# pytorch/ELF

Hardware: AMD Instinct MI355X
Metric: mcts_rollouts_per_sec (self-play, 19x19 Go, 8192 rollouts/move, bs 16) (higher is better)
Workload: dtype f32; 1 GPU; BASELINE configs[2]: MCTS self-play bs=16, 8192 rollouts/move, 20x256 fp16 net on PyTorch-ROCm, 2048 games/GPU in 1 group(s), window crosses a move boundary; games_per_gpu=2048, groups=1, board_size=19, mcts_threads=1, net_dtype=fp16, moves_in_window=2048, nodes_per_game=12288, node_bytes=6626, live_nodes=6241478, largest_tree=8184

## Files before the change

### elf_amd/csrc/net_conv3x3.hip

```cpp
#include <hip/hip_runtime.h>
#include <stdint.h>

#include <atomic>

#include "../../include/elf_amd.h"


namespace {

typedef _Float16 half8 __attribute__((ext_vector_type(8)));
typedef _Float16 half4 __attribute__((ext_vector_type(4)));
typedef float floatx16 __attribute__((ext_vector_type(16)));

constexpr int kTileM = 256;
constexpr int kTileN = 256;
constexpr int kThreads = 512;
constexpr int kOperandBytes = 256 * 128;
constexpr int kBufBytes = 2 * kOperandBytes;
constexpr int kWaveCBytes = 4096;
constexpr int kLdsBytes = 2 * kBufBytes + 8 * kWaveCBytes;

__device__ __attribute__((aligned(128))) unsigned char g_zero_line[128] = {0};

typedef const __attribute__((address_space(1))) void* gptr_t;
typedef __attribute__((address_space(3))) void* lptr_t;

__device__ __forceinline__ void stage16(const char* src, char* lds_base) {
  __builtin_amdgcn_global_load_lds((gptr_t)src, (lptr_t)lds_base, 16, 0, 0);
}

template <int kN, bool kLgkm>
__device__ __forceinline__ void wait_staged() {
  if constexpr (kLgkm) asm volatile("s_waitcnt vmcnt(%0) lgkmcnt(0)" ::"n"(kN) : "memory");
  else asm volatile("s_waitcnt vmcnt(%0)" ::"n"(kN) : "memory");
}
__device__ __forceinline__ void raw_barrier() {
  __builtin_amdgcn_s_barrier();
  asm volatile("" ::: "memory");
  __builtin_amdgcn_sched_barrier(0);
}
template <int kV> struct Mode { static constexpr int v = kV; };
__device__ __forceinline__ int fresh(int v) {
  asm volatile("" : "+v"(v));
  return v;
}
__device__ __forceinline__ int fresh_uniform(int v) {
  asm volatile("" : "+s"(v));
  return v;
}

struct WorkItem { int tile, col, half; };
__host__ __device__ inline WorkItem work_item(int id, int tiles, int nfull) {
  int half = -1;
  if (id >= nfull) {
    const int e = id - nfull;
    id = nfull + (e >> 1);
    half = e & 1;
  }
  const int col = id / tiles;
  return WorkItem{id - col * tiles, col, half};
}
__host__ __device__ inline int full_items(int64_t total, int64_t width) {
  const int64_t r = total % width;
  return (int)(total >= width && r > 0 && 2 * r <= width ? total - r : total);
}

struct Ctx {
  char* lds;
  const char* x;
  const char* w;
  int M, H, W, Cin, K, relu;
  int lane, wv;
  const unsigned char* zsrc;
};
struct Rows { uint32_t xoff[4], woff[4], xmask[4]; };

template <int kNT>
__device__ __forceinline__ void decode_rows(const Ctx& c, Rows& rw, int tile, int kbase) {
  const int lane = c.lane, wv = c.wv;
  const int hw = fresh_uniform(c.H * c.W), wd = fresh_uniform(c.W);
#pragma unroll
  for (int j = 0; j < 4; ++j) {
    const int hf = j >> 1, i = j & 1;
    const int r = i * 128 + hf * 64 + wv * 8 + (lane >> 3);
    const int p = tile * kTileM + r;
    uint32_t m = 0;
    if (p < c.M) {
      const int rem = p % hw, hh = rem / wd, ww = rem - hh * wd;
#pragma unroll
      for (int tap = 0; tap < 9; ++tap) {
        const int dy = tap / 3 - 1, dx = tap % 3 - 1;
        if ((unsigned)(hh + dy) < (unsigned)c.H && (unsigned)(ww + dx) < (unsigned)c.W) m |= 1u << tap;
      }
    }
    rw.xmask[j] = m;
    rw.xoff[j] = (uint32_t)p * (uint32_t)(c.Cin * 2) + (((lane & 7) ^ ((r >> 1) & 7)) << 4);
    const int rwt = kNT == 2 ? (i * 2 + (wv >> 2)) * 64 + hf * 32 + (wv & 3) * 8 + (lane >> 3) : i * 64 + wv * 8 + (lane >> 3);
    rw.woff[j] = (uint32_t)(kbase + rwt) * (uint32_t)(9 * c.Cin * 2) + (((lane & 7) ^ ((rwt >> 1) & 7)) << 4);
  }
}
__device__ __forceinline__ void stage_x(const Ctx& c, const Rows& rw, int hf, int tap, int kc, int buf) {
  const int dy = tap / 3 - 1, dx = tap - (tap / 3) * 3 - 1;
  const uint32_t d = (uint32_t)((dy * c.W + dx) * c.Cin * 2 + kc * 128);
#pragma unroll
  for (int i = 0; i < 2; ++i)
    stage16(((rw.xmask[hf * 2 + i] >> tap) & 1) ? c.x + (uint32_t)(rw.xoff[hf * 2 + i] + d) : (const char*)c.zsrc,
            c.lds + buf * kBufBytes + (i * 128 + hf * 64 + c.wv * 8) * 128);
}
template <int kNT>
__device__ __forceinline__ void stage_w(const Ctx& c, const Rows& rw, int hf, int tap, int kc, int buf) {
  const uint32_t d = (uint32_t)(tap * c.Cin * 2 + kc * 128);
#pragma unroll
  for (int i = 0; i < 2; ++i)
    stage16(c.w + (uint32_t)(rw.woff[hf * 2 + i] + d),
            c.lds + buf * kBufBytes + kOperandBytes +
                (kNT == 2 ? (i * 2 + (c.wv >> 2)) * 64 + hf * 32 + (c.wv & 3) * 8 : i * 64 + c.wv * 8) * 128);
}
struct KPos { int tap1, kc1, tap2, kc2; };
__device__ __forceinline__ KPos first_kpos(int kchunks) {
  KPos k{0, 1, 0, 2};
  if (kchunks == 1) { k.tap1 = 1; k.kc1 = 0; k.tap2 = 2; k.kc2 = 0; }
  else if (kchunks == 2) { k.tap2 = 1; k.kc2 = 0; }
  return k;
}
template <int kNT>
__device__ __forceinline__ void issue_prologue(const Ctx& c, const Rows& rw, int kchunks) {
  const KPos k = first_kpos(fresh_uniform(kchunks));
  stage_x(c, rw, 0, 0, 0, 0); stage_w<kNT>(c, rw, 0, 0, 0, 0);
  if constexpr (kNT == 2) stage_w<kNT>(c, rw, 1, 0, 0, 0);
  stage_x(c, rw, 1, 0, 0, 0);
  stage_x(c, rw, 0, k.tap1, k.kc1, 1); stage_w<kNT>(c, rw, 0, k.tap1, k.kc1, 1);
  if constexpr (kNT == 2) stage_w<kNT>(c, rw, 1, k.tap1, k.kc1, 1);
}

template <int kNT>
__device__ __forceinline__ void main_loop(const Ctx& c, const Rows& rw, floatx16 (&acc)[4][kNT]) {
  char* const lds = c.lds;
  const int lane = c.lane, wv = c.wv;
  const int wm = wv >> 2, wn = wv & 3;
  const int fr = lane & 31, fh = lane >> 5;
  const int sw = (fr >> 1) & 7;
  const int xrow = (wm * 128 + fr) * 128;
  const int wrow = kOperandBytes + (wn * 32 * kNT + fr) * 128;
  int cs[4];
#pragma unroll
  for (int kk = 0; kk < 4; ++kk) cs[kk] = (((kk >> 1) * 4 + fh * 2 + (kk & 1)) ^ sw) << 4;
  auto ldx = [&](const char* b, int mt, int kk) { return *(const half8*)(b + xrow + mt * 4096 + cs[kk]); };
  auto ldw = [&](const char* b, int nt, int kk) { return *(const half8*)(b + wrow + nt * 4096 + cs[kk]); };

#pragma unroll
  for (int mt = 0; mt < 4; ++mt)
#pragma unroll
    for (int nt = 0; nt < kNT; ++nt)
#pragma unroll
      for (int e = 0; e < 16; ++e) acc[mt][nt][e] = 0.0f;

  constexpr int kFly = 2 * (2 + kNT);
  const int kchunks = c.Cin >> 6, ktiles = 9 * kchunks;
  half8 xf[2][4], wa[4], wb[kNT == 2 ? 4 : 1];
  KPos k = first_kpos(kchunks);

  auto ktile = [&](auto mode, int t) {
    constexpr int kMode = decltype(mode)::v;
    const int cur = t & 1, nxt = cur ^ 1;
    const char* b = lds + cur * kBufBytes;
#pragma unroll
    for (int kk = 0; kk < 4; ++kk) {
      wa[kk] = ldw(b, 0, kk);
      xf[0][kk] = ldx(b, 0, kk);
      xf[1][kk] = ldx(b, 1, kk);
      if constexpr (kNT == 2) wb[kk] = ldw(b, 1, kk);
    }
    if constexpr (kMode <= 1) stage_x(c, rw, 1, k.tap1, k.kc1, nxt);
    wait_staged<kMode == 2 ? 0 : kFly, true>();
    raw_barrier();
    __builtin_amdgcn_s_setprio(1);
#pragma unroll
    for (int kk = 0; kk < 4; ++kk) {
      acc[0][0] = __builtin_amdgcn_mfma_f32_32x32x16_f16(wa[kk], xf[0][kk], acc[0][0], 0, 0, 0);
      acc[1][0] = __builtin_amdgcn_mfma_f32_32x32x16_f16(wa[kk], xf[1][kk], acc[1][0], 0, 0, 0);
      if constexpr (kNT == 2) {
        acc[0][1] = __builtin_amdgcn_mfma_f32_32x32x16_f16(wb[kk], xf[0][kk], acc[0][1], 0, 0, 0);
        acc[1][1] = __builtin_amdgcn_mfma_f32_32x32x16_f16(wb[kk], xf[1][kk], acc[1][1], 0, 0, 0);
      }
    }
    __builtin_amdgcn_s_setprio(0);
    __builtin_amdgcn_sched_barrier(0);
    raw_barrier();
#pragma unroll
    for (int kk = 0; kk < 4; ++kk) {
      xf[0][kk] = ldx(b, 2, kk);
      xf[1][kk] = ldx(b, 3, kk);
    }
    if constexpr (kMode == 0) {
      stage_x(c, rw, 0, k.tap2, k.kc2, cur); stage_w<kNT>(c, rw, 0, k.tap2, k.kc2, cur);
      if constexpr (kNT == 2) stage_w<kNT>(c, rw, 1, k.tap2, k.kc2, cur);
    }
    wait_staged<kMode == 0 ? kFly : kMode == 1 ? 2 : 0, true>();
    raw_barrier();
    __builtin_amdgcn_s_setprio(1);
#pragma unroll
    for (int kk = 0; kk < 4; ++kk) {
      acc[2][0] = __builtin_amdgcn_mfma_f32_32x32x16_f16(wa[kk], xf[0][kk], acc[2][0], 0, 0, 0);
      acc[3][0] = __builtin_amdgcn_mfma_f32_32x32x16_f16(wa[kk], xf[1][kk], acc[3][0], 0, 0, 0);
      if constexpr (kNT == 2) {
        acc[2][1] = __builtin_amdgcn_mfma_f32_32x32x16_f16(wb[kk], xf[0][kk], acc[2][1], 0, 0, 0);
        acc[3][1] = __builtin_amdgcn_mfma_f32_32x32x16_f16(wb[kk], xf[1][kk], acc[3][1], 0, 0, 0);
      }
    }
    __builtin_amdgcn_s_setprio(0);
    __builtin_amdgcn_sched_barrier(0);
    raw_barrier();
  };
  const int late = __builtin_amdgcn_readfirstlane(threadIdx.x >> 8);
  if (late) raw_barrier();
  for (int t = 0; t < ktiles - 2; ++t) {
    ktile(Mode<0>{}, t);
    k.tap1 = k.tap2; k.kc1 = k.kc2;
    if (++k.kc2 == kchunks) { k.kc2 = 0; ++k.tap2; }
  }
  ktile(Mode<1>{}, ktiles - 2);
  ktile(Mode<2>{}, ktiles - 1);
  if (!late) raw_barrier();
}

template <bool kHasRes, int kNT>
struct Skip { half8 bv; half8 rv[kHasRes ? 8 * kNT : 1]; };

template <int kNT>
struct EpiLane {
  static constexpr int kC = 4 * kNT;
  static constexpr int kPos = 64 / kC;
  static constexpr int kR = 32 / kPos;
  int pr, q, chan;
  int row0;
  __device__ __forceinline__ EpiLane(const Ctx& c, int tile, int kbase)
      : pr(c.lane / kC), q(c.lane % kC), chan(kbase + (c.wv & 3) * 32 * kNT + (c.lane % kC) * 8),
        row0(tile * kTileM + (c.wv >> 2) * 128) {}
  static __device__ __forceinline__ int swz(int p) { return kNT == 2 ? (p >> 1) & 7 : (p >> 2) & 3; }
};

template <bool kHasRes, int kNT>
__device__ __forceinline__ void load_bias(const Ctx& c, Skip<kHasRes, kNT>& s, const _Float16* __restrict__ bias, int tile, int kbase) {
  const EpiLane<kNT> e(c, tile, kbase);
  s.bv = *(const half8*)(bias + e.chan);
}
template <bool kHasRes, int kNT>
__device__ __forceinline__ void load_skip(const Ctx& c, Skip<kHasRes, kNT>& s, const _Float16* __restrict__ res, int tile, int kbase) {
  using E = EpiLane<kNT>;
  const E e(c, tile, kbase);
  if constexpr (kHasRes) {
#pragma unroll
    for (int it = 0; it < 4 * E::kR; ++it) {
      const int p = e.row0 + (it / E::kR) * 32 + (it % E::kR) * E::kPos + e.pr;
      s.rv[it] = *(const half8*)(res + (size_t)(p < c.M ? p : c.M - 1) * c.K + e.chan);
    }
  }
}

template <bool kHasRes, int kNT, bool kAll>
__device__ __forceinline__ void epilogue(const Ctx& c, const half4 (&hacc)[4][kNT][4], const Skip<kHasRes, kNT>& s,
                                         _Float16* __restrict__ y, int tile, int kbase) {
  using E = EpiLane<kNT>;
  const E e(c, tile, kbase);
  char* const cl = c.lds + 2 * kBufBytes + c.wv * kWaveCBytes;
  const int fr = c.lane & 31, fh = c.lane >> 5;
  constexpr int kRowB = 16 * E::kC;
#pragma unroll
  for (int mt = 0; mt < 4; ++mt) {
#pragma unroll
    for (int nt = 0; nt < kNT; ++nt)
#pragma unroll
      for (int g = 0; g < 4; ++g) *(half4*)(cl + fr * kRowB + (((nt * 4 + g) ^ E::swz(fr)) << 4) + fh * 8) = hacc[mt][nt][g];
    asm volatile("s_waitcnt lgkmcnt(0)" ::: "memory");
#pragma unroll
    for (int j = 0; j < E::kR; ++j) {
      const int pos = j * E::kPos + e.pr;
      const int p = e.row0 + mt * 32 + pos;
      const half8 cv = *(const half8*)(cl + pos * kRowB + ((e.q ^ E::swz(pos)) << 4));
      half8 ov;
#pragma unroll
      for (int i = 0; i < 8; ++i) {
        float v = (float)cv[i];
        v += (float)s.bv[i];
        if constexpr (kHasRes) v += (float)s.rv[mt * E::kR + j][i];
        if (c.relu) v = fmaxf(v, 0.0f);
        ov[i] = (_Float16)v;
      }
      if (kAll || p < c.M) *(half8*)(y + (size_t)p * c.K + e.chan) = ov;
    }
    __builtin_amdgcn_wave_barrier();
  }
}

template <bool kHasRes, int kNT, int kNext>
__device__ __forceinline__ void finish_item(Ctx& c, int lane, Rows& rw, const floatx16 (&acc)[4][kNT], const _Float16* __restrict__ bias,
                                            const _Float16* __restrict__ res, _Float16* __restrict__ y, int tile, int kbase,
                                            int ntile, int nkbase) {
  Skip<kHasRes, kNT> s;
  load_bias<kHasRes, kNT>(c, s, bias, tile, kbase);
  __builtin_amdgcn_sched_barrier(0);
  half4 hacc[4][kNT][4];
#pragma unroll
  for (int mt = 0; mt < 4; ++mt)
#pragma unroll
    for (int nt = 0; nt < kNT; ++nt)
#pragma unroll
      for (int g = 0; g < 4; ++g) {
#pragma unroll
        for (int i = 0; i < 4; ++i) hacc[mt][nt][g][i] = (_Float16)acc[mt][nt][g * 4 + i];
        asm volatile("" : "+v"(hacc[mt][nt][g]));
      }
  c.lane = fresh(lane);
  __builtin_amdgcn_sched_barrier(0);
  load_skip<kHasRes, kNT>(c, s, res, tile, kbase);
  __builtin_amdgcn_sched_barrier(0);
  if constexpr (kNext != 0) {
    decode_rows<kNext>(c, rw, ntile, nkbase);
    __builtin_amdgcn_sched_barrier(0);
  }
  asm volatile("" ::"v"(s.bv));
  if constexpr (kHasRes) {
#pragma unroll
    for (int it = 0; it < 8 * kNT; ++it) asm volatile("" ::"v"(s.rv[it]));
  }
  if constexpr (kNext != 0) {
    issue_prologue<kNext>(c, rw, c.Cin >> 6);
    __builtin_amdgcn_sched_barrier(0);
  }
  const bool all = __builtin_amdgcn_readfirstlane((tile + 1) * kTileM <= c.M);
  if (all) epilogue<kHasRes, kNT, true>(c, hacc, s, y, tile, kbase);
  else epilogue<kHasRes, kNT, false>(c, hacc, s, y, tile, kbase);
  if constexpr (kNext != 0) {
    constexpr int kFly = 2 * (2 + kNext);
    if (all) wait_staged<kFly + 8 * kNT, false>();
    else wait_staged<kFly, false>();
    raw_barrier();
  }
}

template <bool kHasRes>
__global__ __launch_bounds__(kThreads, 2) void k_conv3x3_f16(const char* __restrict__ x, const char* __restrict__ w,
                                                             const _Float16* __restrict__ bias, const _Float16* __restrict__ res,
                                                             _Float16* __restrict__ y, int M, int H, int W, int Cin, int K, int relu,
                                                             int tiles, int nfull, int ids) {
  __shared__ __attribute__((aligned(128))) char lds[kLdsBytes];
  const int tid = threadIdx.x;
  Ctx c;
  c.lds = lds; c.x = x; c.w = w; c.M = M; c.H = H; c.W = W; c.Cin = Cin; c.K = K; c.relu = relu;
  c.lane = tid & 63;
  c.wv = __builtin_amdgcn_readfirstlane(tid >> 6);
  c.zsrc = g_zero_line + (c.lane & 7) * 16;
  const int G = (int)gridDim.x;
  int id = (int)blockIdx.x;
  WorkItem wi = work_item(id, tiles, nfull);
  Rows rw;
  decode_rows<2>(c, rw, wi.tile, wi.col * kTileN);
  issue_prologue<2>(c, rw, Cin >> 6);
  wait_staged<8, false>();
  raw_barrier();
  const int lane = c.lane;
  int hk = 0;
  for (;;) {
    floatx16 acc[4][2];
    c.lane = fresh(lane);
    main_loop<2>(c, rw, acc);
    const int nid = id + G;
    if (nid >= ids) {
      finish_item<kHasRes, 2, 0>(c, lane, rw, acc, bias, res, y, wi.tile, wi.col * kTileN, 0, 0);
      return;
    }
    const WorkItem nwi = work_item(nid, tiles, nfull);
    if (__builtin_amdgcn_readfirstlane(nwi.half) >= 0) {
      const int nkbase = nwi.col * kTileN + nwi.half * (kTileN / 2);
      finish_item<kHasRes, 2, 1>(c, lane, rw, acc, bias, res, y, wi.tile, wi.col * kTileN, nwi.tile, nkbase);
      wi = nwi; hk = nkbase;
      break;
    }
    finish_item<kHasRes, 2, 2>(c, lane, rw, acc, bias, res, y, wi.tile, wi.col * kTileN, nwi.tile, nwi.col * kTileN);
    id = nid;
    wi = nwi;
  }
  floatx16 acch[4][1];
  c.lane = fresh(lane);
  main_loop<1>(c, rw, acch);
  finish_item<kHasRes, 1, 0>(c, lane, rw, acch, bias, res, y, wi.tile, hk, 0, 0);
}

int round_width_of_device() {
  static std::atomic<int> cus[64];
  int dev = 0;
  if (hipGetDevice(&dev) != hipSuccess || dev < 0 || dev >= 64) { (void)hipGetLastError(); return 0; }
  int n = cus[dev].load(std::memory_order_relaxed);
  if (n == 0) {
    if (hipDeviceGetAttribute(&n, hipDeviceAttributeMultiprocessorCount, dev) != hipSuccess || n <= 0) { (void)hipGetLastError(); return 0; }
    cus[dev].store(n, std::memory_order_relaxed);
  }
  return n;
}

}

extern "C" __attribute__((visibility("hidden"))) int elfnet_conv3x3_native_f16(const void* x, const void* w, const void* bias,
                                                                               const void* res, void* y, int64_t rows, int h, int wd,
                                                                               int c, int k, int relu, int round_width,
                                                                               hipStream_t stream) {
  if ((c & 63) != 0 || (k & 255) != 0 || round_width < 0) return ELFGO_E_BADARG;
  const int64_t m = rows * h * wd;
  const int tiles = (int)((m + kTileM - 1) / kTileM), cols = k / kTileN;
  const int64_t total = (int64_t)tiles * cols;
  const int width = round_width > 0 ? round_width : round_width_of_device();
  const int nfull = width > 0 ? full_items(total, width) : (int)total;
  const int64_t ids = 2 * total - nfull;
  const dim3 grid((unsigned)(width > 0 && width < ids ? width : ids));
  if (res)
    hipLaunchKernelGGL(k_conv3x3_f16<true>, grid, dim3(kThreads), 0, stream, (const char*)x, (const char*)w, (const _Float16*)bias,
                       (const _Float16*)res, (_Float16*)y, (int)m, h, wd, c, k, relu, tiles, nfull, (int)ids);
  else
    hipLaunchKernelGGL(k_conv3x3_f16<false>, grid, dim3(kThreads), 0, stream, (const char*)x, (const char*)w, (const _Float16*)bias,
                       (const _Float16*)nullptr, (_Float16*)y, (int)m, h, wd, c, k, relu, tiles, nfull, (int)ids);
  hipError_t e = hipGetLastError();
  return e == hipSuccess ? 0 : (int)e;
}

extern "C" int64_t elfnet_conv3x3_f16_plan(int64_t tiles, int columns, int round_width, int64_t id, int* tile, int* column, int* half) {
  if (tiles <= 0 || columns <= 0 || round_width <= 0 || tiles * columns >= ((int64_t)1 << 30)) return ELFGO_E_BADARG;
  const int64_t total = tiles * columns;
  const int nfull = full_items(total, round_width);
  const int64_t groups = 2 * total - nfull;
  if (tile || column || half) {
    if (id < 0 || id >= groups) return ELFGO_E_BADARG;
    const WorkItem wi = work_item((int)id, (int)tiles, nfull);
    if (tile) *tile = wi.tile;
    if (column) *column = wi.col;
    if (half) *half = wi.half;
  }
  return groups;
}

extern "C" int64_t elfnet_conv3x3_f16_grid(int64_t tiles, int columns, int round_width) {
  const int64_t ids = elfnet_conv3x3_f16_plan(tiles, columns, round_width, 0, nullptr, nullptr, nullptr);
  return ids < 0 ? ids : round_width < ids ? round_width : ids;
}
```

Before: 63870 rollouts/s.

## Interleave global-to-LDS staging loads between MFMA instructions in conv3x3 mainloop

Splits the per-k-tile async global-to-LDS staging into individual 16-byte pieces and issues them at fixed positions inside the MFMA sequence of each half-tile, instead of issuing them all in a burst before each MFMA block. The aim is to spread memory-issue work across matrix-core execution so both units stay busy and the issue bursts stop stalling the MFMA stream. Wait counts are retuned to match the new issue order, and a compile-time macro selects among priority strategies (the default keeps per-segment setprio). The risk is wrong vmcnt accounting or sched_barrier constraints that hurt the compiler's scheduling.

```diff
diff --git a/elf_amd/csrc/net_conv3x3.hip b/elf_amd/csrc/net_conv3x3.hip
--- a/elf_amd/csrc/net_conv3x3.hip
+++ b/elf_amd/csrc/net_conv3x3.hip
@@ -40,6 +40,9 @@
   __builtin_amdgcn_sched_barrier(0);
 }
 template <int kV> struct Mode { static constexpr int v = kV; };
+#ifndef ELFNET_CONV3X3_PRIO
+#define ELFNET_CONV3X3_PRIO 0
+#endif
 __device__ __forceinline__ int fresh(int v) {
   asm volatile("" : "+v"(v));
   return v;
@@ -99,22 +102,31 @@
     rw.woff[j] = (uint32_t)(kbase + rwt) * (uint32_t)(9 * c.Cin * 2) + (((lane & 7) ^ ((rwt >> 1) & 7)) << 4);
   }
 }
+__device__ __forceinline__ uint32_t x_delta(const Ctx& c, int tap, int kc) {
+  const int dy = tap / 3 - 1, dx = tap - (tap / 3) * 3 - 1;
+  return (uint32_t)((dy * c.W + dx) * c.Cin * 2 + kc * 128);
+}
+__device__ __forceinline__ uint32_t w_delta(const Ctx& c, int tap, int kc) { return (uint32_t)(tap * c.Cin * 2 + kc * 128); }
+__device__ __forceinline__ void stage_x_piece(const Ctx& c, const Rows& rw, int hf, int i, int tap, uint32_t d, int buf) {
+  stage16(((rw.xmask[hf * 2 + i] >> tap) & 1) ? c.x + (uint32_t)(rw.xoff[hf * 2 + i] + d) : (const char*)c.zsrc,
+          c.lds + buf * kBufBytes + (i * 128 + hf * 64 + c.wv * 8) * 128);
+}
+template <int kNT>
+__device__ __forceinline__ void stage_w_piece(const Ctx& c, const Rows& rw, int hf, int i, uint32_t d, int buf) {
+  stage16(c.w + (uint32_t)(rw.woff[hf * 2 + i] + d),
+          c.lds + buf * kBufBytes + kOperandBytes +
+              (kNT == 2 ? (i * 2 + (c.wv >> 2)) * 64 + hf * 32 + (c.wv & 3) * 8 : i * 64 + c.wv * 8) * 128);
+}
 __device__ __forceinline__ void stage_x(const Ctx& c, const Rows& rw, int hf, int tap, int kc, int buf) {
-  const int dy = tap / 3 - 1, dx = tap - (tap / 3) * 3 - 1;
-  const uint32_t d = (uint32_t)((dy * c.W + dx) * c.Cin * 2 + kc * 128);
-#pragma unroll
-  for (int i = 0; i < 2; ++i)
-    stage16(((rw.xmask[hf * 2 + i] >> tap) & 1) ? c.x + (uint32_t)(rw.xoff[hf * 2 + i] + d) : (const char*)c.zsrc,
-            c.lds + buf * kBufBytes + (i * 128 + hf * 64 + c.wv * 8) * 128);
+  const uint32_t d = x_delta(c, tap, kc);
+#pragma unroll
+  for (int i = 0; i < 2; ++i) stage_x_piece(c, rw, hf, i, tap, d, buf);
 }
 template <int kNT>
 __device__ __forceinline__ void stage_w(const Ctx& c, const Rows& rw, int hf, int tap, int kc, int buf) {
-  const uint32_t d = (uint32_t)(tap * c.Cin * 2 + kc * 128);
-#pragma unroll
-  for (int i = 0; i < 2; ++i)
-    stage16(c.w + (uint32_t)(rw.woff[hf * 2 + i] + d),
-            c.lds + buf * kBufBytes + kOperandBytes +
-                (kNT == 2 ? (i * 2 + (c.wv >> 2)) * 64 + hf * 32 + (c.wv & 3) * 8 : i * 64 + c.wv * 8) * 128);
+  const uint32_t d = w_delta(c, tap, kc);
+#pragma unroll
+  for (int i = 0; i < 2; ++i) stage_w_piece<kNT>(c, rw, hf, i, d, buf);
 }
 struct KPos { int tap1, kc1, tap2, kc2; };
 __device__ __forceinline__ KPos first_kpos(int kchunks) {
@@ -155,15 +167,55 @@
 #pragma unroll
       for (int e = 0; e < 16; ++e) acc[mt][nt][e] = 0.0f;
 
-  constexpr int kFly = 2 * (2 + kNT);
+  constexpr int kWaitL1 = 2 * (1 + kNT), kWaitL2 = 2;
+  constexpr int kM1At[2] = {4 * kNT - 1, 6 * kNT - 1};
+  constexpr int kM2At[6] = {2 * kNT - 1, 2 * kNT + 1, 2 * kNT + 3, kNT == 2 ? 9 : 6, 11, 13};
   const int kchunks = c.Cin >> 6, ktiles = 9 * kchunks;
   half8 xf[2][4], wa[4], wb[kNT == 2 ? 4 : 1];
   KPos k = first_kpos(kchunks);
+  auto wfrag = [&](int nt, int kk) -> half8 {
+    if constexpr (kNT == 2) return nt ? wb[kk] : wa[kk];
+    else return wa[kk];
+  };
+
+  auto mseg = [&](auto seg, auto pieces, int cur, int tap, uint32_t dx, uint32_t dw) {
+    constexpr int kSeg = decltype(seg)::v, kP = decltype(pieces)::v;
+#if ELFNET_CONV3X3_PRIO == 0
+    __builtin_amdgcn_s_setprio(1);
+#endif
+#pragma unroll
+    for (int kk = 0; kk < 4; ++kk)
+#pragma unroll
+      for (int nt = 0; nt < kNT; ++nt)
+#pragma unroll
+        for (int m = 0; m < 2; ++m) {
+          acc[2 * kSeg + m][nt] = __builtin_amdgcn_mfma_f32_32x32x16_f16(wfrag(nt, kk), xf[m][kk], acc[2 * kSeg + m][nt], 0, 0, 0);
+          const int at = (kk * kNT + nt) * 2 + m;
+#pragma unroll
+          for (int p = 0; p < kP; ++p)
+            if (at == (kSeg == 0 ? kM1At[p] : kM2At[p])) {
+              __builtin_amdgcn_sched_barrier(0);
+              if constexpr (kSeg == 0) stage_x_piece(c, rw, 1, p, tap, dx, cur ^ 1);
+              else if (p < 2) stage_x_piece(c, rw, 0, p, tap, dx, cur);
+              else stage_w_piece<kNT>(c, rw, (p - 2) >> 1, p & 1, dw, cur);
+              __builtin_amdgcn_sched_barrier(0);
+            }
+        }
+#if ELFNET_CONV3X3_PRIO == 0
+    __builtin_amdgcn_s_setprio(0);
+#endif
+    __builtin_amdgcn_sched_barrier(0);
+    raw_barrier();
+  };
 
   auto ktile = [&](auto mode, int t) {
     constexpr int kMode = decltype(mode)::v;
-    const int cur = t & 1, nxt = cur ^ 1;
+    const int cur = t & 1;
     const char* b = lds + cur * kBufBytes;
+    uint32_t dx1 = 0, dx2 = 0, dw2 = 0;
+    if constexpr (kMode <= 1) dx1 = x_delta(c, k.tap1, k.kc1);
+    if constexpr (kMode == 0) { dx2 = x_delta(c, k.tap2, k.kc2); dw2 = w_delta(c, k.tap2, k.kc2); }
+    asm volatile("" : "+s"(dx1), "+s"(dx2), "+s"(dw2));
 #pragma unroll
     for (int kk = 0; kk < 4; ++kk) {
       wa[kk] = ldw(b, 0, kk);
@@ -171,49 +223,23 @@
       xf[1][kk] = ldx(b, 1, kk);
       if constexpr (kNT == 2) wb[kk] = ldw(b, 1, kk);
     }
-    if constexpr (kMode <= 1) stage_x(c, rw, 1, k.tap1, k.kc1, nxt);
-    wait_staged<kMode == 2 ? 0 : kFly, true>();
+    wait_staged<kMode == 2 ? 0 : kWaitL1, true>();
     raw_barrier();
-    __builtin_amdgcn_s_setprio(1);
-#pragma unroll
-    for (int kk = 0; kk < 4; ++kk) {
-      acc[0][0] = __builtin_amdgcn_mfma_f32_32x32x16_f16(wa[kk], xf[0][kk], acc[0][0], 0, 0, 0);
-      acc[1][0] = __builtin_amdgcn_mfma_f32_32x32x16_f16(wa[kk], xf[1][kk], acc[1][0], 0, 0, 0);
-      if constexpr (kNT == 2) {
-        acc[0][1] = __builtin_amdgcn_mfma_f32_32x32x16_f16(wb[kk], xf[0][kk], acc[0][1], 0, 0, 0);
-        acc[1][1] = __builtin_amdgcn_mfma_f32_32x32x16_f16(wb[kk], xf[1][kk], acc[1][1], 0, 0, 0);
-      }
-    }
-    __builtin_amdgcn_s_setprio(0);
-    __builtin_amdgcn_sched_barrier(0);
-    raw_barrier();
+    mseg(Mode<0>{}, Mode<kMode <= 1 ? 2 : 0>{}, cur, k.tap1, dx1, 0);
 #pragma unroll
     for (int kk = 0; kk < 4; ++kk) {
       xf[0][kk] = ldx(b, 2, kk);
       xf[1][kk] = ldx(b, 3, kk);
     }
-    if constexpr (kMode == 0) {
-      stage_x(c, rw, 0, k.tap2, k.kc2, cur); stage_w<kNT>(c, rw, 0, k.tap2, k.kc2, cur);
-      if constexpr (kNT == 2) stage_w<kNT>(c, rw, 1, k.tap2, k.kc2, cur);
-    }
-    wait_staged<kMode == 0 ? kFly : kMode == 1 ? 2 : 0, true>();
+    wait_staged<kMode == 2 ? 0 : kWaitL2, true>();
     raw_barrier();
-    __builtin_amdgcn_s_setprio(1);
-#pragma unroll
-    for (int kk = 0; kk < 4; ++kk) {
-      acc[2][0] = __builtin_amdgcn_mfma_f32_32x32x16_f16(wa[kk], xf[0][kk], acc[2][0], 0, 0, 0);
-      acc[3][0] = __builtin_amdgcn_mfma_f32_32x32x16_f16(wa[kk], xf[1][kk], acc[3][0], 0, 0, 0);
-      if constexpr (kNT == 2) {
-        acc[2][1] = __builtin_amdgcn_mfma_f32_32x32x16_f16(wb[kk], xf[0][kk], acc[2][1], 0, 0, 0);
-        acc[3][1] = __builtin_amdgcn_mfma_f32_32x32x16_f16(wb[kk], xf[1][kk], acc[3][1], 0, 0, 0);
-      }
-    }
-    __builtin_amdgcn_s_setprio(0);
-    __builtin_amdgcn_sched_barrier(0);
-    raw_barrier();
+    mseg(Mode<1>{}, Mode<kMode == 0 ? 2 + 2 * kNT : 0>{}, cur, k.tap2, dx2, dw2);
   };
   const int late = __builtin_amdgcn_readfirstlane(threadIdx.x >> 8);
   if (late) raw_barrier();
+#if ELFNET_CONV3X3_PRIO == 2
+  if (late) __builtin_amdgcn_s_setprio(1);
+#endif
   for (int t = 0; t < ktiles - 2; ++t) {
     ktile(Mode<0>{}, t);
     k.tap1 = k.tap2; k.kc1 = k.kc2;
@@ -221,6 +247,9 @@
   }
   ktile(Mode<1>{}, ktiles - 2);
   ktile(Mode<2>{}, ktiles - 1);
+#if ELFNET_CONV3X3_PRIO == 2
+  __builtin_amdgcn_s_setprio(0);
+#endif
   if (!late) raw_barrier();
 }
 
```

New measurement: 65150 rollouts/s, median of 6. 2.0% higher.
